# thvlio/bp-from-video

Hardware: NVIDIA B200
Metric: roi_sampled_frames_per_s (higher is better)
Workload: dtype f64

## Files before the change

bp-from-video_b200/csrc/window_pre.cu:

```cuda
#include <stdlib.h>
#include "filters.cuh"
#include "corr_tile.cuh"

namespace bpv {

int launch_job_butter(const double* ring_t, const bpv_window_params& p, double* sos_out, cudaStream_t st);
int launch_job_firls(const double* ring_t, const bpv_window_params& p, double* taps_out, cudaStream_t st);
int check_filter_params(const bpv_window_params* p, const char* who);
int launch_design_cached(const double* ring_t, const bpv_window_params& p, bool butter, bool fir, unsigned char* cache,
                         int32_t* ref, void* miss, double* ws_sos, double* ws_fir, cudaStream_t st);

struct DesignRef {
  const double* sos_ws;
  const double* taps_ws;
  const int32_t* ref;
  const unsigned char* cache;
  __device__ __forceinline__ const double* slot(long long job) const {
    const int sl = ref ? ref[job] : -1;
    return sl >= 0 ? reinterpret_cast<const double*>(cache + DC_HDR_BYTES + DC_SLOTS * 8) + (long long)sl * DC_STRIDE : nullptr;
  }
  __device__ __forceinline__ const double* sos(long long job) const {
    const double* v = slot(job);
    return v ? v : sos_ws + job * (MAX_SOS * 6);
  }
  __device__ __forceinline__ const double* fir(long long job) const {
    const double* v = slot(job);
    return v ? v + MAX_SOS * 6 : taps_ws + job * FIR_WS_STRIDE;
  }
};

struct PreLayout {
  int yv, xv, posv, posb, buf0, buf1, coef, total;
  int buf_len;
  int fir_c, fir_gt, fir_b;
};

__host__ __device__ inline int round_up(int v, int m) { return (v + m - 1) / m * m; }
__host__ __device__ inline int fir_ld_fwd(int n, int T) {
  int LD = (round_up(T, 8) + n + T + 15) / 8 + 1;
  LD += (6 - (LD & 3)) & 3;
  return LD;
}
__host__ __device__ inline int fir_ld_bwd(int n, int T) { return (round_up(T, 10) + n + T + 20) / 10 + 1; }
__host__ __device__ inline int fir_merged_k(int T, int RT) { return round_up(2 * T - 1, RT); }
__host__ __device__ inline int fir_merged_ld(int n, int T, int RT) { return (fir_merged_k(T, RT) / RT + (n + RT - 1) / RT) | 1; }

__host__ __device__ inline PreLayout pre_layout(const bpv_window_params& p, bool taps_global = false) {
  bool interp = false, cubic = false, butter = false, fir = false;
  for (int i = 0; i < p.num_methods; ++i) {
    const int m = p.methods[i];
    interp |= (m == BPV_INTERP_LINEAR || m == BPV_INTERP_CUBIC);
    cubic |= m == BPV_INTERP_CUBIC;
    butter |= m == BPV_FILTER_BUTTER;
    fir |= m == BPV_FILTER_FIR;
  }
  const int W = p.window;
  int pad = 0;
  if (butter) pad = 3 * (2 * p.butter_order + 1);
  if (pad > W - 1) pad = W - 1 > 0 ? W - 1 : 0;
  PreLayout L;
  L.buf_len = butter ? W + 2 * pad : (interp ? W : 0);
  L.fir_c = L.fir_gt = L.fir_b = 0;
  if (fir) {
    const int T = p.fir_taps, nf = W < T - 1 ? W : T - 1;
    L.fir_gt = 8 * fir_ld_fwd(nf, T);
    L.fir_b = L.fir_gt + 10 * fir_ld_bwd(nf, T);
    int need = L.fir_b;
    if (W >= T) {
      const int x8 = 8 * fir_merged_ld(W, T, 8), x10 = 10 * fir_merged_ld(W, T, 10);
      L.fir_c = ((x8 > x10 ? x8 : x10) + 1) & ~1;
      const int k8 = fir_merged_k(T, 8), k10 = fir_merged_k(T, 10);
      const int m = L.fir_c + (taps_global ? 0 : (k8 > k10 ? k8 : k10));
      if (m > need) need = m;
    }
    if (need > L.buf_len) L.buf_len = need;
  }
  int o = 0;
  auto sect = [&o](int bytes) { const int at = o; o += (bytes + 15) / 16 * 16; return at; };
  L.yv = sect(W * 8);
  L.xv = sect(interp ? W * 8 : 0);
  L.buf0 = sect(L.buf_len * 8);
  L.buf1 = sect(cubic ? W * 8 : 0);
  L.coef = sect(butter ? 128 * 8 : 0);
  L.posv = sect(W * 2);
  L.posb = sect(interp ? W * 2 : 0);
  L.total = o;
  return L;
}

__device__ __forceinline__ double shfl_d(double v, int src) { return __shfl_sync(0xffffffffu, v, src); }
__device__ __forceinline__ double shfl_up_d(double v, int d) { return __shfl_up_sync(0xffffffffu, v, d); }

struct Warp {
  int lane;
  double *yv, *xv, *buf0, *buf1, *coef;
  unsigned short *posv, *posb;
  int n, m;
  double xfirst, xlast;
  bool grid;
  int fir_c, fir_gt, fir_b;
  int W;
};

__device__ void diff1(Warp& w) {
  for (int c = (w.n - 1) / 32; c >= 0; --c) {
    const int i = c * 32 + w.lane;
    double v = 0.0;
    if (i < w.n && i > 0) v = w.yv[i] - w.yv[i - 1];
    __syncwarp();
    if (i < w.n) w.yv[i] = v;
    __syncwarp();
  }
}

__device__ void diff2(Warp& w) {
  const double y0 = w.yv[0], y1 = w.yv[1];
  __syncwarp();
  for (int c = (w.n - 1) / 32; c >= 0; --c) {
    const int i = c * 32 + w.lane;
    double v = 0.0;
    if (i < w.n) {
      const double z2 = w.yv[i];
      const double z1 = i >= 1 ? w.yv[i - 1] : y1;
      const double z0 = i >= 2 ? w.yv[i - 2] : (i == 1 ? y1 : y0);
      v = (z2 - z1) - (z1 - z0);
    }
    __syncwarp();
    if (i < w.n) w.yv[i] = v;
    __syncwarp();
  }
}

__device__ void detrend_const(Warp& w) {
  double s = 0.0;
  for (int i = w.lane; i < w.n; i += 32) s += w.yv[i];
  const double mean = warp_sum(s) / (double)w.n;
  for (int i = w.lane; i < w.n; i += 32) w.yv[i] -= mean;
  __syncwarp();
}

__device__ void detrend_linear(Warp& w) {
  const double N = (double)w.n, invN = 1.0 / N;
  double s = 0.0;
  for (int i = w.lane; i < w.n; i += 32) s += w.yv[i];
  const double ybar = warp_sum(s) * invN;
  const double ubar = (N + 1.0) * 0.5 * invN;
  double sxy = 0.0;
  for (int i = w.lane; i < w.n; i += 32) {
    const double du = fma((double)(i + 1), invN, -ubar);
    sxy = fma(du, w.yv[i] - ybar, sxy);
  }
  sxy = warp_sum(sxy);
  const double sxx = (N * N - 1.0) / (12.0 * N);
  const double slope = sxx > 0.0 ? sxy / sxx : 0.0;
  for (int i = w.lane; i < w.n; i += 32) {
    const double du = fma((double)(i + 1), invN, -ubar);
    w.yv[i] = (w.yv[i] - ybar) - slope * du;
  }
  __syncwarp();
}

__device__ __forceinline__ double grid_x(const Warp& w, int i, double step) {
  if (i == w.m - 1 && w.m > 1) return w.xlast;
  return __dadd_rn(__dmul_rn((double)i, step), w.xfirst);
}

__device__ __forceinline__ int bsearch_le(const double* xs, int n, double x) {
  int lo = 0, hi = n;
  while (hi - lo > 1) {
    const int mid = (lo + hi) >> 1;
    if (xs[mid] <= x) lo = mid; else hi = mid;
  }
  return lo;
}

__device__ void finish_interp(Warp& w, double step) {
  __syncwarp();
  for (int i = w.lane; i < w.m; i += 32) {
    w.yv[i] = w.buf0[i];
    w.xv[i] = grid_x(w, i, step);
    w.posv[i] = w.posb[i];
  }
  w.n = w.m;
  w.grid = true;
  __syncwarp();
}

__device__ void interp_linear(Warp& w) {
  const double step = (w.xlast - w.xfirst) / (double)(w.m - 1);
  const int n = w.n;
  for (int i = w.lane; i < w.m; i += 32) {
    const double xi = grid_x(w, i, step);
    double r;
    if (xi > w.xv[n - 1]) r = w.yv[n - 1];
    else if (xi < w.xv[0]) r = w.yv[0];
    else {
      const int j = bsearch_le(w.xv, n, xi);
      if (j == n - 1 || w.xv[j] == xi) r = w.yv[j];
      else {
        const double slope = (w.yv[j + 1] - w.yv[j]) / (w.xv[j + 1] - w.xv[j]);
        r = __dadd_rn(__dmul_rn(slope, xi - w.xv[j]), w.yv[j]);
      }
    }
    w.buf0[i] = r;
  }
  finish_interp(w, step);
}

__device__ bool interp_cubic(Warp& w) {
  const int n = w.n;
  const double* x = w.xv;
  const double* y = w.yv;
  int bad = 0;
  for (int i = w.lane; i + 1 < n; i += 32) bad |= !(x[i + 1] - x[i] > 0.0);
  if (__any_sync(0xffffffffu, bad)) return false;
  double* cp = w.buf0;
  double* s = w.buf1;
  if (w.lane == 0) {
    if (n == 2) {
      s[0] = s[1] = (y[1] - y[0]) / (x[1] - x[0]);
    } else if (n == 3) {
      const double dx0 = x[1] - x[0], dx1 = x[2] - x[1];
      const double sl0 = (y[1] - y[0]) / dx0, sl1 = (y[2] - y[1]) / dx1;
      const double s1 = (dx0 * sl1 + dx1 * sl0) / (dx0 + dx1);
      s[1] = s1; s[0] = 2.0 * sl0 - s1; s[2] = 2.0 * sl1 - s1;
    }
  }
  if (n > 3) {
    for (int i = 1 + w.lane; i <= n - 2; i += 32) {
      const double dxp = x[i] - x[i - 1], dxc = x[i + 1] - x[i];
      const double slp = (y[i] - y[i - 1]) / dxp, slc = (y[i + 1] - y[i]) / dxc;
      cp[i] = 2.0 * (dxp + dxc);
      s[i] = 3.0 * (dxc * slp + dxp * slc);
    }
    __syncwarp();
    if (w.lane == 0) {
      double cprev, sprev;
      {
        const double dx0 = x[1] - x[0], dx1 = x[2] - x[1];
        const double sl0 = (y[1] - y[0]) / dx0, sl1 = (y[2] - y[1]) / dx1;
        const double d = x[2] - x[0];
        const double rhs = ((dx0 + 2.0 * d) * dx1 * sl0 + dx0 * dx0 * sl1) / d;
        const double inv = 1.0 / dx1;
        cprev = d * inv; sprev = rhs * inv;
        cp[0] = cprev; s[0] = sprev;
      }
      double xm = x[0], xc = x[1], xn = x[2];
#pragma unroll 4
      for (int i = 1; i <= n - 2; ++i) {
        const double lo = xn - xc, up = xc - xm;
        const double inv = 1.0 / fma(-lo, cprev, cp[i]);
        cprev = up * inv;
        sprev = fma(-lo, sprev, s[i]) * inv;
        cp[i] = cprev; s[i] = sprev;
        xm = xc; xc = xn; xn = x[i + 2 < n ? i + 2 : n - 1];
      }
      {
        const double dxp = x[n - 2] - x[n - 3], dxc = x[n - 1] - x[n - 2];
        const double slp = (y[n - 2] - y[n - 3]) / dxp, slc = (y[n - 1] - y[n - 2]) / dxc;
        const double d = x[n - 1] - x[n - 3];
        const double rhs = (dxc * dxc * slp + (2.0 * d + dxc) * dxp * slc) / d;
        const double den = dxp - d * cprev;
        double sn = (rhs - d * sprev) / den;
        s[n - 1] = sn;
#pragma unroll 4
        for (int i = n - 2; i >= 0; --i) { sn = fma(-cp[i], sn, s[i]); s[i] = sn; }
      }
    }
  }
  __syncwarp();
  const double step = (w.xlast - w.xfirst) / (double)(w.m - 1);
  for (int i = w.lane; i < w.m; i += 32) {
    const double xi = grid_x(w, i, step);
    int j;
    if (xi < x[0]) j = 0;
    else if (xi >= x[n - 1]) j = n - 2;
    else j = bsearch_le(x, n, xi);
    const double dxj = x[j + 1] - x[j];
    const double slj = (y[j + 1] - y[j]) / dxj;
    const double t = (s[j] + s[j + 1] - 2.0 * slj) / dxj;
    const double c0 = t / dxj, c1 = (slj - s[j]) / dxj - t, c2 = s[j], c3 = y[j];
    const double u = xi - x[j];
    double res = c3, z = u;
    res = __dadd_rn(res, __dmul_rn(c2, z)); z = __dmul_rn(z, u);
    res = __dadd_rn(res, __dmul_rn(c1, z)); z = __dmul_rn(z, u);
    res = __dadd_rn(res, __dmul_rn(c0, z));
    cp[i] = res;
  }
  finish_interp(w, step);
  return true;
}

__device__ void odd_ext(const Warp& w, double* ext, int p) {
  const int n = w.n, L = n + 2 * p;
  const double y0 = w.yv[0], yl = w.yv[n - 1];
  for (int i = w.lane; i < L; i += 32) {
    double v;
    if (i < p) v = 2.0 * y0 - w.yv[p - i];
    else if (i < p + n) v = w.yv[i - p];
    else v = 2.0 * yl - w.yv[n - 2 - (i - p - n)];
    ext[i] = v;
  }
  __syncwarp();
}

__device__ void sos_filtfilt(Warp& w, const double* __restrict__ sos_g, int N) {
  double* sos = w.coef;
  double* zi = w.coef + 6 * MAX_SOS;
  for (int i = w.lane; i < N * 6; i += 32) sos[i] = sos_g[i];
  __syncwarp();
  int nb0 = 0, na0 = 0;
  if (w.lane == 0) {
    double scale = 1.0;
    for (int s = 0; s < N; ++s) {
      const double* c = sos + 6 * s;
      const double B0 = c[1] - c[4] * c[0], B1 = c[2] - c[5] * c[0];
      const double z0 = (B0 + B1) / (1.0 + c[4] + c[5]);
      zi[2 * s] = scale * z0;
      zi[2 * s + 1] = scale * (B1 - c[5] * z0);
      scale *= (c[0] + c[1] + c[2]) / (1.0 + c[4] + c[5]);
    }
  }
  for (int s = 0; s < N; ++s) { nb0 += sos[6 * s + 2] == 0.0; na0 += sos[6 * s + 5] == 0.0; }
  __syncwarp();
  const int dpl = 3 * (2 * N + 1 - (nb0 < na0 ? nb0 : na0));
  const int n = w.n, p = n <= dpl ? n - 1 : dpl;
  const int L = n + 2 * p;
  double* ext = w.buf0;
  odd_ext(w, ext, p);

  const int s = w.lane;
  const bool sec = s < N;
  const double b0 = sec ? sos[6 * s] : 0, b1 = sec ? sos[6 * s + 1] : 0, b2 = sec ? sos[6 * s + 2] : 0;
  const double a1 = sec ? sos[6 * s + 4] : 0, a2 = sec ? sos[6 * s + 5] : 0;
  const double zi0 = sec ? zi[2 * s] : 0, zi1 = sec ? zi[2 * s + 1] : 0;

  const double na1 = -a1, na2 = -a2;
  for (int pass = 0; pass < 2; ++pass) {
    const double x0 = pass == 0 ? ext[0] : ext[L - 1];
    double z0 = zi0 * x0, z1 = zi1 * x0;
    double prev_out = 0.0;
    const int dir = pass == 0 ? 1 : -1, base = pass == 0 ? 0 : L - 1;
    double nxt = ext[base];
    __syncwarp();
    const int t_steady = N - 1 < L ? N - 1 : L;
    int t = 0;
    for (; t < t_steady; ++t) {
      const double from_prev = shfl_up_d(prev_out, 1);
      const double xc = s == 0 ? nxt : from_prev;
      if (s == 0 && t + 1 < L) nxt = ext[base + dir * (t + 1)];
      if (sec && t >= s) {
        const double xn = fma(b0, xc, z0);
        z0 = fma(b1, xc, fma(na1, xn, z1));
        z1 = fma(b2, xc, na2 * xn);
        prev_out = xn;
      }
    }
    const double* in = ext + base + dir * (t + 1);
    double* out = ext + base + dir * (t - (N - 1));
    for (; t < L - 1; ++t) {
      const double from_prev = shfl_up_d(prev_out, 1);
      const double xc = s == 0 ? nxt : from_prev;
      if (s == 0) nxt = *in;
      in += dir;
      const double xn = fma(b0, xc, z0);
      z0 = fma(b1, xc, fma(na1, xn, z1));
      z1 = fma(b2, xc, na2 * xn);
      prev_out = xn;
      if (s == N - 1) *out = xn;
      out += dir;
    }
    for (; t < L + N - 1; ++t) {
      const double from_prev = shfl_up_d(prev_out, 1);
      const double xc = s == 0 ? nxt : from_prev;
      const int i = t - s;
      if (sec && i >= 0 && i < L) {
        const double xn = fma(b0, xc, z0);
        z0 = fma(b1, xc, fma(na1, xn, z1));
        z1 = fma(b2, xc, na2 * xn);
        prev_out = xn;
        if (s == N - 1) ext[base + dir * i] = xn;
      }
    }
    __syncwarp();
  }
  for (int i = w.lane; i < n; i += 32) w.yv[i] = ext[p + i];
  __syncwarp();
}

__device__ void sos_filtfilt_dual(Warp& wa, Warp& wb, bool la, bool lb, const double* __restrict__ ga,
                                  const double* __restrict__ gb, int N) {
  const int lane = wa.lane, hf = lane >> 4, s = lane & 15;
  const bool live = hf ? lb : la;
  double* yv = hf ? wb.yv : wa.yv;
  double* ext = hf ? wb.buf0 : wa.buf0;
  double* sos = hf ? wb.coef : wa.coef;
  double* zi = sos + 6 * MAX_SOS;
  const double* sg = hf ? gb : ga;
  const int n = live ? (hf ? wb.n : wa.n) : 0;
  if (live) for (int i = s; i < N * 6; i += 16) sos[i] = sg[i];
  __syncwarp();
  int nb0 = 0, na0 = 0;
  if (live) {
    if (s == 0) {
      double scale = 1.0;
      for (int k = 0; k < N; ++k) {
        const double* c = sos + 6 * k;
        const double B0 = c[1] - c[4] * c[0], B1 = c[2] - c[5] * c[0];
        const double z0 = (B0 + B1) / (1.0 + c[4] + c[5]);
        zi[2 * k] = scale * z0;
        zi[2 * k + 1] = scale * (B1 - c[5] * z0);
        scale *= (c[0] + c[1] + c[2]) / (1.0 + c[4] + c[5]);
      }
    }
    for (int k = 0; k < N; ++k) { nb0 += sos[6 * k + 2] == 0.0; na0 += sos[6 * k + 5] == 0.0; }
  }
  __syncwarp();
  const int dpl = 3 * (2 * N + 1 - (nb0 < na0 ? nb0 : na0));
  const int p = n <= dpl ? n - 1 : dpl;
  const int L = live ? n + 2 * p : 0;
  if (live) {
    const double y0 = yv[0], yl = yv[n - 1];
    for (int i = s; i < L; i += 16) {
      double v;
      if (i < p) v = 2.0 * y0 - yv[p - i];
      else if (i < p + n) v = yv[i - p];
      else v = 2.0 * yl - yv[n - 2 - (i - p - n)];
      ext[i] = v;
    }
  }
  __syncwarp();
  const int La = __shfl_sync(0xffffffffu, L, 0), Lb = __shfl_sync(0xffffffffu, L, 16);
  const int Lmax = La > Lb ? La : Lb;
  const int Lfast = (La > 0 && Lb > 0) ? (La < Lb ? La : Lb) : Lmax;
  const bool sec = live && s < N;
  const double b0 = sec ? sos[6 * s] : 0, b1 = sec ? sos[6 * s + 1] : 0, b2 = sec ? sos[6 * s + 2] : 0;
  const double a1 = sec ? sos[6 * s + 4] : 0, a2 = sec ? sos[6 * s + 5] : 0;
  const double zi0 = sec ? zi[2 * s] : 0, zi1 = sec ? zi[2 * s + 1] : 0;
  const double na1 = -a1, na2 = -a2;
  const bool first = live && s == 0, last = live && s == N - 1;
  for (int pass = 0; pass < 2; ++pass) {
    const double x0 = L > 0 ? (pass == 0 ? ext[0] : ext[L - 1]) : 0.0;
    double z0 = zi0 * x0, z1 = zi1 * x0;
    double prev_out = 0.0;
    const int dir = pass == 0 ? 1 : -1, base = pass == 0 ? 0 : L - 1;
    double nxt = L > 0 ? ext[base] : 0.0;
    __syncwarp();
    const int t_fill = N - 1 < Lmax ? N - 1 : Lmax;
    int t = 0;
    for (; t < t_fill; ++t) {
      const double from_prev = __shfl_up_sync(0xffffffffu, prev_out, 1, 16);
      const double xc = s == 0 ? nxt : from_prev;
      if (first && t + 1 < L) nxt = ext[base + dir * (t + 1)];
      if (sec && t >= s && t - s < L) {
        const double xn = fma(b0, xc, z0);
        z0 = fma(b1, xc, fma(na1, xn, z1));
        z1 = fma(b2, xc, na2 * xn);
        prev_out = xn;
        if (s == N - 1) ext[base + dir * (t - s)] = xn;
      }
    }
    if (Lfast > 0) {
      const double* in = ext + (L > 0 ? base + dir * (t + 1) : 0);
      double* out = ext + (L > 0 ? base + dir * (t - (N - 1)) : 0);
      for (; t < Lfast - 1; ++t) {
        const double from_prev = __shfl_up_sync(0xffffffffu, prev_out, 1, 16);
        const double xc = s == 0 ? nxt : from_prev;
        if (first) nxt = *in;
        in += dir;
        const double xn = fma(b0, xc, z0);
        z0 = fma(b1, xc, fma(na1, xn, z1));
        z1 = fma(b2, xc, na2 * xn);
        prev_out = xn;
        if (last) *out = xn;
        out += dir;
      }
    }
    for (; t < Lmax + N - 1; ++t) {
      const double from_prev = __shfl_up_sync(0xffffffffu, prev_out, 1, 16);
      const double xc = s == 0 ? nxt : from_prev;
      if (first && t + 1 < L) nxt = ext[base + dir * (t + 1)];
      const int i = t - s;
      if (sec && i >= 0 && i < L) {
        const double xn = fma(b0, xc, z0);
        z0 = fma(b1, xc, fma(na1, xn, z1));
        z1 = fma(b2, xc, na2 * xn);
        prev_out = xn;
        if (s == N - 1) ext[base + dir * i] = xn;
      }
    }
    __syncwarp();
  }
  if (live) for (int i = s; i < n; i += 16) yv[i] = ext[p + i];
  __syncwarp();
}

constexpr int FIR_RT = 8;
constexpr int FIR_RTB = 10;
__device__ void fir_filtfilt(Warp& w, const double* __restrict__ taps_g, int T) {
  const int Kp = (T + FIR_RT - 1) / FIR_RT * FIR_RT;
  const int KpB = (T + FIR_RTB - 1) / FIR_RTB * FIR_RTB;
  const double* __restrict__ b = taps_g;
  const double* __restrict__ zi = taps_g + 128;
  const int n = w.n, dpl = 3 * T, p = n <= dpl ? n - 1 : dpl;
  const int L = n + 2 * p;
  const int fa = p, fb = (p + n - 1 + T - 1) < (L - 1) ? (p + n - 1 + T - 1) : (L - 1);
  const int ba = p, bb = p + n - 1;
  const int xbase = fa - Kp, gbase = ba - KpB;
  int LD = (Kp + n + T + 15) / FIR_RT + 1;
  LD += (6 - (LD & 3)) & 3;
  const int LDB = (KpB + n + T + 2 * FIR_RTB) / FIR_RTB + 1;
  double* XT = w.buf0;
  double* GT = w.buf0 + w.fir_gt;
  const double y_first = w.yv[0], y_last = w.yv[n - 1];
#pragma unroll 3
  for (int jj = w.lane; jj < FIR_RT * LD; jj += 32) {
    const int i = jj + xbase;
    const bool inside = i >= 0 && i < L, head = i < p, tail = i >= p + n;
    const int src = head ? p - i : (tail ? 2 * n - 2 + p - i : i - p);
    const double y = w.yv[inside ? src : 0];
    const double v = head ? 2.0 * y_first - y : (tail ? 2.0 * y_last - y : y);
    XT[xt_index<FIR_RT>(jj, LD)] = inside ? v : 0.0;
  }
#pragma unroll 4
  for (int jj = w.lane; jj < FIR_RTB * LDB; jj += 32) GT[jj] = 0.0;
  __syncwarp();
  const double x0 = p >= 1 ? 2.0 * y_first - w.yv[p] : y_first;
  for (int I = Kp; I <= fb - xbase; I += 32 * FIR_RT) {
    const int j0 = I + FIR_RT * w.lane, i0 = j0 + xbase;
    if (i0 <= fb) {
      double acc[FIR_RT];
#pragma unroll
      for (int r = 0; r < FIR_RT; ++r) acc[r] = 0.0;
      corr_tile<FIR_RT, double, 0, 0, true>(acc, b, Kp, XT, LD, j0, 0, 0x7fffffff, T);
#pragma unroll
      for (int r = 0; r < FIR_RT; ++r) {
        const int i = i0 + r;
        if (i <= fb) {
          const double v = acc[r] + (i < T - 1 ? zi[i] * x0 : 0.0);
          const int g = L - 1 - i;
          GT[xt_index<FIR_RTB>(g - gbase, LDB)] = v;
        }
      }
    }
  }
  __syncwarp();
  const double yend = (0 - gbase >= 0) ? GT[xt_index<FIR_RTB>(0 - gbase, LDB)] : 0.0;
  for (int I = KpB; I <= bb - gbase; I += 32 * FIR_RTB) {
    const int j0 = I + FIR_RTB * w.lane, i0 = j0 + gbase;
    if (i0 <= bb) {
      double acc[FIR_RTB];
#pragma unroll
      for (int r = 0; r < FIR_RTB; ++r) acc[r] = 0.0;
      corr_tile<FIR_RTB, double, 0, 0, true>(acc, b, KpB, GT, LDB, j0, 0, 0x7fffffff, T);
#pragma unroll
      for (int r = 0; r < FIR_RTB; ++r) {
        const int i = i0 + r;
        if (i <= bb) w.yv[L - 1 - p - i] = acc[r] + (i < T - 1 ? zi[i] * yend : 0.0);
      }
    }
  }
  __syncwarp();
}

template <int RT, int LDC = 0, int KC = 0, bool CS = true>
__device__ void fir_merged(Warp& w, const double* __restrict__ c_g, int T) {
  const int M = T - 1;
  const int K = KC ? KC : fir_merged_k(T, RT);
  const int n = w.n, dpl = 3 * T, p = n <= dpl ? n - 1 : dpl;
  const int L = n + 2 * p;
  const int tiles = (n + RT - 1) / RT;
  const int LD = LDC ? LDC : fir_merged_ld(w.W, T, RT);
  double* XT = w.buf0;
  const double* c = c_g;
  if (CS) {
    double* cs = w.buf0 + w.fir_c;
    for (int k = w.lane; k < K; k += 32) cs[k] = c_g[k];
    c = cs;
  }
  const int xbase = p + M - K;
  const double y_first = w.yv[0], y_last = w.yv[n - 1];
  const int total = RT * (K / RT + tiles);
  const int j_h = xbase < 0 ? -xbase : 0;
  const int j_b = p - xbase, j_t = p + n - xbase;
  const int j_e = L - xbase < total ? L - xbase : total;
  for (int jj = w.lane; jj < j_h; jj += 32) XT[xt_index<RT>(jj, LD)] = 0.0;
  for (int jj = j_h + w.lane; jj < j_b; jj += 32) XT[xt_index<RT>(jj, LD)] = 2.0 * y_first - w.yv[j_b - jj];
  for (int jj = j_b + w.lane; jj < j_t && jj < total; jj += 32) XT[xt_index<RT>(jj, LD)] = w.yv[jj - j_b];
  for (int jj = j_t + w.lane; jj < j_e; jj += 32) XT[xt_index<RT>(jj, LD)] = 2.0 * y_last - w.yv[2 * n - 2 - (jj - j_b)];
  for (int jj = (j_e > j_t ? j_e : j_t) + w.lane; jj < total; jj += 32) XT[xt_index<RT>(jj, LD)] = 0.0;
  __syncwarp();
  for (int t = w.lane; t < tiles; t += 32) {
    double acc[RT];
#pragma unroll
    for (int r = 0; r < RT; ++r) acc[r] = 0.0;
    corr_tile<RT, double, LDC, KC>(acc, c, K, XT, LD, K + RT * t);
#pragma unroll
    for (int r = 0; r < RT; ++r) {
      const int m = RT * t + r;
      if (m < n) w.yv[m] = acc[r];
    }
  }
  __syncwarp();
}

template <bool CS>
__device__ __forceinline__ void fir_apply(Warp& w, const double* __restrict__ tg, int T) {
  const int n = w.n;
  if (n >= T) {
    const int c8 = ((n + 7) / 8 + 31) / 32 * 8 * fir_merged_k(T, 8);
    const int c10 = ((n + 9) / 10 + 31) / 32 * 10 * fir_merged_k(T, 10);
    const bool t127 = T == 127;
    if (c10 < c8) {
      if (t127 && w.W == 300) fir_merged<10, 57, 260, CS>(w, tg + 256, T);
      else fir_merged<10, 0, 0, CS>(w, tg + 256, T);
    } else {
      if (t127 && w.W == 300) fir_merged<8, 71, 256, CS>(w, tg + 256, T);
      else if (t127 && w.W == 250) fir_merged<8, 65, 256, CS>(w, tg + 256, T);
      else fir_merged<8, 0, 0, CS>(w, tg + 256, T);
    }
  } else {
    fir_filtfilt(w, tg, T);
  }
}

constexpr int F_INTERP = 1, F_BUTTER = 2, F_FIR = 4;
constexpr int F_TAPS_GLOBAL = 8;

__device__ __forceinline__ bool fs_is_finite(double xfirst, double xlast, int m) {
  const double d = fabs(xlast - xfirst);
  if (d > 1.0e-290 && d < 1.0e290) return true;
  return isfinite(1.0 / ((xlast - xfirst) / (double)(m - 1)));
}

template <int FEAT>
__device__ int gather_window(Warp& w, unsigned char* sm, const PreLayout& L, const bpv_window_params& p,
                             const double* __restrict__ ring_t, const double* __restrict__ ring_y, long long sig,
                             double* __restrict__ ox, double* __restrict__ oy) {
  bool has_interp = false;
  if (FEAT & F_INTERP)
    for (int i = 0; i < p.num_methods; ++i) has_interp |= (p.methods[i] == BPV_INTERP_LINEAR || p.methods[i] == BPV_INTERP_CUBIC);
  w.yv = reinterpret_cast<double*>(sm + L.yv);
  w.xv = reinterpret_cast<double*>(sm + L.xv);
  w.buf0 = reinterpret_cast<double*>(sm + L.buf0);
  w.buf1 = reinterpret_cast<double*>(sm + L.buf1);
  w.coef = reinterpret_cast<double*>(sm + L.coef);
  w.posv = reinterpret_cast<unsigned short*>(sm + L.posv);
  w.posb = reinterpret_cast<unsigned short*>(sm + L.posb);
  w.grid = false;
  w.W = p.window;
  w.fir_c = L.fir_c; w.fir_gt = L.fir_gt; w.fir_b = L.fir_b;
  const long long job = sig / p.R;
  const int r = (int)(sig % p.R);
  const int s = (int)(job / p.jobs_per_stream), j = (int)(job % p.jobs_per_stream);
  const long long head = p.head0 + (long long)j * p.head_step;
  const double* rt = ring_t + (long long)s * p.cap;
  const double* ry = ring_y + ((long long)s * p.R + r) * p.cap;
  const int W = p.window;
  int n = 0, m = 0;
  double xfirst = 0.0, xlast = 0.0;
  const unsigned lt = (1u << w.lane) - 1u;
  const long long gfirst = head - W + 1;
  const int kmin = gfirst < 0 ? (int)(-gfirst < W ? -gfirst : W) : 0;
  const int slot0 = (int)(((gfirst % p.cap) + p.cap) % p.cap);
  double* xstage = L.buf_len >= W ? w.buf0 : nullptr;
  bool allf = true;
  for (int k = w.lane; k < W; k += 32) {
    double x = nan_f64(), y = nan_f64();
    if (k >= kmin) { int slot = slot0 + k; if (slot >= p.cap) slot -= p.cap; x = rt[slot]; y = ry[slot]; }
    ox[k] = x; oy[k] = y;
    w.yv[k] = y;
    if (xstage) xstage[k] = x;
    allf &= isfinite(x) && isfinite(y);
  }
  __syncwarp();
  if (xstage && !has_interp && __all_sync(0xffffffffu, allf)) {
    for (int k = w.lane; k < W; k += 32) w.posv[k] = (unsigned short)k;
    w.n = w.m = W;
    w.xfirst = xstage[0]; w.xlast = xstage[W - 1];
    __syncwarp();
    return (W >= 2 && fs_is_finite(w.xfirst, w.xlast, W)) ? ST_OK : ST_GUARD;
  }
  for (int k0 = 0; k0 < W; k0 += 32) {
    const int k = k0 + w.lane;
    double x = nan_f64(), y = nan_f64();
    if (k < W) {
      y = w.yv[k];
      if (xstage) x = xstage[k];
      else if (k >= kmin) { int slot = slot0 + k; if (slot >= p.cap) slot -= p.cap; x = rt[slot]; }
    }
    const bool fx = isfinite(x), fy = isfinite(y);
    const unsigned bx = __ballot_sync(0xffffffffu, fx), by = __ballot_sync(0xffffffffu, fy);
    __syncwarp();
    if (fy) {
      const int idx = n + __popc(by & lt);
      w.yv[idx] = y; w.posv[idx] = (unsigned short)k;
      if (has_interp) w.xv[idx] = x;
    }
    if (fx && has_interp) w.posb[m + __popc(bx & lt)] = (unsigned short)k;
    if (bx) {
      if (m == 0) xfirst = shfl_d(x, __ffs(bx) - 1);
      xlast = shfl_d(x, 31 - __clz(bx));
    }
    __syncwarp();
    n += __popc(by); m += __popc(bx);
  }
  __syncwarp();
  w.n = n; w.m = m; w.xfirst = xfirst; w.xlast = xlast;
  return (n >= 2 && m >= 2 && fs_is_finite(xfirst, xlast, m)) ? ST_OK : ST_GUARD;
}

template <int FEAT>
__device__ int apply_method(Warp& w, int method, const bpv_window_params& p, const DesignRef& dr, long long job) {
  switch (method) {
    case BPV_DIFF_1: diff1(w); break;
    case BPV_DIFF_2: diff2(w); break;
    case BPV_INTERP_LINEAR: if (FEAT & F_INTERP) interp_linear(w); break;
    case BPV_INTERP_CUBIC: if (FEAT & F_INTERP) { if (!interp_cubic(w)) return ST_CUBIC_X; } break;
    case BPV_DETREND_CONST: detrend_const(w); break;
    case BPV_DETREND_LINEAR: detrend_linear(w); break;
    case BPV_FILTER_BUTTER:
      if (FEAT & F_BUTTER) {
        const double* sg = dr.sos(job);
        if (!isfinite(sg[0])) return ST_BAD_BANDS;
        sos_filtfilt(w, sg, p.butter_order);
      }
      break;
    case BPV_FILTER_FIR:
      if (FEAT & F_FIR) {
        const double* tg = dr.fir(job);
        if (!isfinite(tg[0])) return ST_BAD_BANDS;
        fir_apply<(FEAT & F_TAPS_GLOBAL) == 0>(w, tg, p.fir_taps);
      }
      break;
    default: break;
  }
  return ST_OK;
}

__device__ void scatter_window(const Warp& w, int st, int W, double* __restrict__ ox, double* __restrict__ oy,
                               int32_t* __restrict__ status, long long sig) {
  if (st == ST_OK) {
    for (int i = w.lane; i < w.n; i += 32) {
      const int k = w.posv[i];
      oy[k] = w.yv[i];
      if (w.grid) ox[k] = w.xv[i];
    }
  } else if (st != ST_GUARD) {
    for (int k = w.lane; k < W; k += 32) oy[k] = nan_f64();
  }
  if (w.lane == 0) status[sig] = st;
}

__device__ __forceinline__ void prefetch_filters(int FEAT, int lane, const bpv_window_params& p, const DesignRef& dr, long long job) {
  for (int i = 0; i < p.num_methods; ++i) {
    if ((FEAT & F_FIR) && p.methods[i] == BPV_FILTER_FIR) {
      asm volatile("prefetch.global.L1 [%0];" ::"l"(dr.fir(job) + lane * 16));
      if (lane == 0) asm volatile("prefetch.global.L1 [%0];" ::"l"(dr.fir(job) + 512));
    }
    if ((FEAT & F_BUTTER) && p.methods[i] == BPV_FILTER_BUTTER && lane * 16 < p.butter_order * 6)
      asm volatile("prefetch.global.L1 [%0];" ::"l"(dr.sos(job) + lane * 16));
  }
}

template <int FEAT, int MINB, bool DUAL>
__global__ void __launch_bounds__(128, MINB) window_preprocess_kernel(const double* __restrict__ ring_t,
                                                                      const double* __restrict__ ring_y,
                                                                      const bpv_window_params p, const PreLayout L,
                                                                      const DesignRef dr,
                                                                      double* __restrict__ proc_x, double* __restrict__ proc_y,
                                                                      int32_t* __restrict__ status) {
  extern __shared__ __align__(16) unsigned char smem_raw[];
  const int wib = threadIdx.x >> 5, wpb = blockDim.x >> 5;
  const long long unit = (long long)blockIdx.x * wpb + wib;
  const long long nsig = (long long)p.S * p.jobs_per_stream * p.R;
  const int W = p.window;
  const int lane = threadIdx.x & 31;
  if (!DUAL) {
    const long long sig = unit;
    if (sig >= nsig) return;
    Warp w;
    w.lane = lane;
    const long long job = sig / p.R;
    prefetch_filters(FEAT, lane, p, dr, job);
    double* ox = proc_x + sig * W;
    double* oy = proc_y + sig * W;
    int st = gather_window<FEAT>(w, smem_raw + (size_t)wib * L.total, L, p, ring_t, ring_y, sig, ox, oy);
    for (int mi = 0; mi < p.num_methods && st == ST_OK; ++mi) st = apply_method<FEAT>(w, p.methods[mi], p, dr, job);
    scatter_window(w, st, W, ox, oy, status, sig);
  } else {
    const long long sa = 2 * unit, sb = sa + 1;
    if (sa >= nsig) return;
    const bool hasb = sb < nsig;
    Warp wa, wb;
    wa.lane = wb.lane = lane;
    const long long ja = sa / p.R, jb = (hasb ? sb : sa) / p.R;
    prefetch_filters(FEAT, lane, p, dr, ja);
    if (jb != ja) prefetch_filters(FEAT, lane, p, dr, jb);
    unsigned char* sm = smem_raw + (size_t)wib * 2 * L.total;
    double* oxa = proc_x + sa * W; double* oya = proc_y + sa * W;
    double* oxb = proc_x + (hasb ? sb : sa) * W; double* oyb = proc_y + (hasb ? sb : sa) * W;
    int sta = gather_window<FEAT>(wa, sm, L, p, ring_t, ring_y, sa, oxa, oya);
    int stb = ST_GUARD;
    if (hasb) stb = gather_window<FEAT>(wb, sm + L.total, L, p, ring_t, ring_y, sb, oxb, oyb);
    else { wb = wa; }
    for (int mi = 0; mi < p.num_methods && (sta == ST_OK || stb == ST_OK); ++mi) {
      const int m = p.methods[mi];
      if (m == BPV_FILTER_BUTTER) {
        const double* ga = dr.sos(ja);
        const double* gb = dr.sos(jb);
        if (sta == ST_OK && !isfinite(ga[0])) sta = ST_BAD_BANDS;
        if (stb == ST_OK && !isfinite(gb[0])) stb = ST_BAD_BANDS;
        if (sta == ST_OK || stb == ST_OK) sos_filtfilt_dual(wa, wb, sta == ST_OK, stb == ST_OK, ga, gb, p.butter_order);
      } else {
        if (sta == ST_OK) sta = apply_method<FEAT & ~F_BUTTER>(wa, m, p, dr, ja);
        if (stb == ST_OK) stb = apply_method<FEAT & ~F_BUTTER>(wb, m, p, dr, jb);
      }
    }
    scatter_window(wa, sta, W, oxa, oya, status, sa);
    if (hasb) scatter_window(wb, stb, W, oxb, oyb, status, sb);
  }
}

template <int FEAT, int MINB, bool DUAL>
static int launch_preprocess(const double* ring_t, const double* ring_y, const bpv_window_params& p, const PreLayout& L,
                             const DesignRef& dr, double* proc_x, double* proc_y, int32_t* status, cudaStream_t st) {
  const int max_smem = 200 * 1024;
  const int per_warp = (DUAL ? 2 : 1) * L.total;
  BPV_REQUIRE(per_warp <= max_smem, BPV_E_TOO_LARGE, "bpv_window_preprocess: window %d needs %d B of shared memory per signal",
              p.window, L.total);
  const int reg_warps = MINB >= 6 ? 25 : (MINB == 5 ? 21 : 4 * MINB);
  int wpb = 1, best = 0;
  for (int c = 1; c <= 4; ++c) {
    const int per_block = c * per_warp + 1024;
    if (per_block > max_smem) break;
    int blocks = (227 * 1024) / per_block;
    if (blocks > 32) blocks = 32;
    int warps = blocks * c;
    if (warps > reg_warps) warps = reg_warps;
    if (warps > best || (warps == best && c < wpb)) { best = warps; wpb = c; }
  }
  const size_t smem = (size_t)wpb * per_warp;
  auto kern = window_preprocess_kernel<FEAT, MINB, DUAL>;
  if (int rc = ensure_dyn_smem((const void*)kern, smem)) return rc;
  const long long nsig = (long long)p.S * p.jobs_per_stream * p.R;
  const long long units = DUAL ? (nsig + 1) / 2 : nsig;
  kern<<<(unsigned)((units + wpb - 1) / wpb), wpb * 32, smem, st>>>(ring_t, ring_y, p, L, dr, proc_x, proc_y, status);
  return check_launch("bpv_window_preprocess");
}

static int parse_methods(const bpv_window_params* p, const char* who, bool& butter, bool& fir, bool& interp) {
  butter = fir = interp = false;
  BPV_REQUIRE(p->num_methods >= 0 && p->num_methods <= BPV_MAX_METHODS, BPV_E_INVALID, "%s: bad sizes", who);
  for (int i = 0; i < p->num_methods; ++i) {
    const int m = p->methods[i];
    BPV_REQUIRE(m >= BPV_DIFF_1 && m <= BPV_FILTER_FIR, BPV_E_UNSUPPORTED,
                "%s: unknown processing method %d (NotImplementedError, signal_processor.py:238)", who, m);
    butter |= m == BPV_FILTER_BUTTER;
    fir |= m == BPV_FILTER_FIR;
    interp |= m == BPV_INTERP_LINEAR || m == BPV_INTERP_CUBIC;
  }
  return 0;
}

}

namespace bpv {
struct WsPlan { long long sos, fir, ref, miss, total; };
static WsPlan ws_plan(const bpv_window_params* p) {
  const long long J = (long long)p->S * p->jobs_per_stream;
  WsPlan w;
  w.sos = 0;
  w.fir = w.sos + J * MAX_SOS * 6 * 8;
  w.ref = w.fir + J * FIR_WS_STRIDE * 8;
  w.miss = w.ref + (J * 4 + 7) / 8 * 8;
  w.total = w.miss + J * 16;
  return w;
}
}

extern "C" int64_t bpv_window_workspace_bytes(const bpv_window_params* p) {
  if (!p) return -1;
  return bpv::ws_plan(p).total;
}

extern "C" int64_t bpv_design_cache_bytes(void) { return bpv::DC_BYTES; }

extern "C" int bpv_window_design(const double* ring_t, const bpv_window_params* p, void* workspace, int64_t workspace_bytes,
                                 void* cache, int64_t cache_bytes, void* stream) {
  using namespace bpv;
  if (int rc = check_filter_params(p, "bpv_window_design")) return rc;
  BPV_REQUIRE(ring_t, BPV_E_INVALID, "bpv_window_design: NULL pointer");
  BPV_REQUIRE(p->S > 0 && p->window > 0 && p->window <= p->cap && p->jobs_per_stream > 0, BPV_E_INVALID, "bpv_window_design: bad sizes");
  bool butter, fir, interp;
  if (int rc = parse_methods(p, "bpv_window_design", butter, fir, interp)) return rc;
  if (!butter && !fir) return 0;
  const WsPlan wp = ws_plan(p);
  BPV_REQUIRE(workspace && workspace_bytes >= wp.total, BPV_E_INVALID,
              "bpv_window_design: workspace too small (see bpv_window_workspace_bytes)");
  BPV_REQUIRE(!cache || cache_bytes >= DC_BYTES, BPV_E_INVALID, "bpv_window_design: design cache too small (see bpv_design_cache_bytes)");
  unsigned char* ws = (unsigned char*)workspace;
  double* sos_ws = (double*)(ws + wp.sos);
  double* taps_ws = (double*)(ws + wp.fir);
  cudaStream_t st = (cudaStream_t)stream;
  if (cache)
    return launch_design_cached(ring_t, *p, butter, fir, (unsigned char*)cache, (int32_t*)(ws + wp.ref), ws + wp.miss, sos_ws, taps_ws, st);
  if (butter) if (int rc = launch_job_butter(ring_t, *p, sos_ws, st)) return rc;
  if (fir) if (int rc = launch_job_firls(ring_t, *p, taps_ws, st)) return rc;
  return 0;
}

extern "C" int bpv_window_filter(const double* ring_t, const double* ring_y, const bpv_window_params* p,
                                 const void* workspace, int64_t workspace_bytes, const void* cache, int64_t cache_bytes,
                                 double* proc_x, double* proc_y, int32_t* status, void* stream) {
  using namespace bpv;
  if (int rc = check_filter_params(p, "bpv_window_preprocess")) return rc;
  BPV_REQUIRE(ring_t && ring_y && proc_x && proc_y && status, BPV_E_INVALID, "bpv_window_preprocess: NULL pointer");
  BPV_REQUIRE(p->S > 0 && p->R > 0 && p->window > 0 && p->window <= p->cap && p->jobs_per_stream > 0, BPV_E_INVALID,
              "bpv_window_preprocess: bad sizes");
  BPV_REQUIRE(p->window <= 65535, BPV_E_TOO_LARGE, "bpv_window_preprocess: window > 65535");
  bool butter, fir, interp;
  if (int rc = parse_methods(p, "bpv_window_preprocess", butter, fir, interp)) return rc;
  const WsPlan wp = ws_plan(p);
  if (butter || fir) {
    BPV_REQUIRE(workspace && workspace_bytes >= wp.total, BPV_E_INVALID,
                "bpv_window_preprocess: workspace too small (see bpv_window_workspace_bytes)");
    BPV_REQUIRE(!cache || cache_bytes >= DC_BYTES, BPV_E_INVALID, "bpv_window_preprocess: design cache too small (see bpv_design_cache_bytes)");
  }
  const unsigned char* ws = (const unsigned char*)workspace;
  DesignRef dr;
  dr.sos_ws = ws ? (const double*)(ws + wp.sos) : nullptr;
  dr.taps_ws = ws ? (const double*)(ws + wp.fir) : nullptr;
  dr.ref = (ws && cache && (butter || fir)) ? (const int32_t*)(ws + wp.ref) : nullptr;
  dr.cache = (const unsigned char*)cache;
  static const bool taps_global = [] { const char* e = getenv("BPV_FIR_TAPS_GLOBAL"); return e && e[0] == '1'; }();
  const bool fir_only = !interp && !butter && fir;
  const PreLayout L = pre_layout(*p, fir_only && taps_global);
  cudaStream_t st = (cudaStream_t)stream;
#define BPV_PRE(feat, minb, dual) return launch_preprocess<feat, minb, dual>(ring_t, ring_y, *p, L, dr, proc_x, proc_y, status, st)
  const bool single_sos = getenv("BPV_SOS_SINGLE") != nullptr || (227 * 1024) / (2 * L.total + 1024) < 8;
  if (!interp && !butter && !fir) BPV_PRE(0, 6, false);
  if (fir_only && taps_global) BPV_PRE(F_FIR | F_TAPS_GLOBAL, 6, false);
  if (fir_only) BPV_PRE(F_FIR, 5, false);
  if (single_sos) {
    if (!interp && !fir) BPV_PRE(F_BUTTER, 4, false);
    BPV_PRE(F_INTERP | F_BUTTER | F_FIR, 4, false);
  }
  if (!interp && !fir) BPV_PRE(F_BUTTER, 4, true);
  if (!fir) BPV_PRE(F_INTERP | F_BUTTER, 4, true);
  BPV_PRE(F_INTERP | F_BUTTER | F_FIR, 4, true);
#undef BPV_PRE
}

extern "C" int bpv_window_preprocess(const double* ring_t, const double* ring_y, const bpv_window_params* p,
                                     void* workspace, int64_t workspace_bytes,
                                     double* proc_x, double* proc_y, int32_t* status, void* stream) {
  if (int rc = bpv_window_design(ring_t, p, workspace, workspace_bytes, nullptr, 0, stream)) return rc;
  return bpv_window_filter(ring_t, ring_y, p, workspace, workspace_bytes, nullptr, 0, proc_x, proc_y, status, stream);
}
```

Measured before the change: 23.67 million.

## Add chunked streaming FIR preprocessing kernel sharing overlapping windows per CTA

```diff
diff --git a/bp-from-video_b200/csrc/window_pre.cu b/bp-from-video_b200/csrc/window_pre.cu
--- a/bp-from-video_b200/csrc/window_pre.cu
+++ b/bp-from-video_b200/csrc/window_pre.cu
@@ -100,6 +100,7 @@
   bool grid;
   int fir_c, fir_gt, fir_b;
   int W;
+  const double* taps;
 };
 
 __device__ void diff1(Warp& w) {
@@ -563,7 +564,7 @@
   __syncwarp();
 }
 
-template <int RT, int LDC = 0, int KC = 0, bool CS = true>
+template <int RT, int LDC = 0, int KC = 0, bool CS = true, bool PRE = false>
 __device__ void fir_merged(Warp& w, const double* __restrict__ c_g, int T) {
   const int M = T - 1;
   const int K = KC ? KC : fir_merged_k(T, RT);
@@ -573,7 +574,9 @@
   const int LD = LDC ? LDC : fir_merged_ld(w.W, T, RT);
   double* XT = w.buf0;
   const double* c = c_g;
-  if (CS) {
+  if (PRE) {
+    c = w.taps;
+  } else if (CS) {
     double* cs = w.buf0 + w.fir_c;
     for (int k = w.lane; k < K; k += 32) cs[k] = c_g[k];
     c = cs;
@@ -604,7 +607,7 @@
   __syncwarp();
 }
 
-template <bool CS>
+template <bool CS, bool PRE = false>
 __device__ __forceinline__ void fir_apply(Warp& w, const double* __restrict__ tg, int T) {
   const int n = w.n;
   if (n >= T) {
@@ -612,12 +615,12 @@
     const int c10 = ((n + 9) / 10 + 31) / 32 * 10 * fir_merged_k(T, 10);
     const bool t127 = T == 127;
     if (c10 < c8) {
-      if (t127 && w.W == 300) fir_merged<10, 57, 260, CS>(w, tg + 256, T);
-      else fir_merged<10, 0, 0, CS>(w, tg + 256, T);
+      if (t127 && w.W == 300) fir_merged<10, 57, 260, CS, PRE>(w, tg + 256, T);
+      else fir_merged<10, 0, 0, CS, PRE>(w, tg + 256, T);
     } else {
-      if (t127 && w.W == 300) fir_merged<8, 71, 256, CS>(w, tg + 256, T);
-      else if (t127 && w.W == 250) fir_merged<8, 65, 256, CS>(w, tg + 256, T);
-      else fir_merged<8, 0, 0, CS>(w, tg + 256, T);
+      if (t127 && w.W == 300) fir_merged<8, 71, 256, CS, PRE>(w, tg + 256, T);
+      else if (t127 && w.W == 250) fir_merged<8, 65, 256, CS, PRE>(w, tg + 256, T);
+      else fir_merged<8, 0, 0, CS, PRE>(w, tg + 256, T);
     }
   } else {
     fir_filtfilt(w, tg, T);
@@ -626,6 +629,7 @@
 
 constexpr int F_INTERP = 1, F_BUTTER = 2, F_FIR = 4;
 constexpr int F_TAPS_GLOBAL = 8;
+constexpr int F_TAPS_CTA = 16;
 
 __device__ __forceinline__ bool fs_is_finite(double xfirst, double xlast, int m) {
   const double d = fabs(xlast - xfirst);
@@ -730,7 +734,7 @@
       if (FEAT & F_FIR) {
         const double* tg = dr.fir(job);
         if (!isfinite(tg[0])) return ST_BAD_BANDS;
-        fir_apply<(FEAT & F_TAPS_GLOBAL) == 0>(w, tg, p.fir_taps);
+        fir_apply<(FEAT & (F_TAPS_GLOBAL | F_TAPS_CTA)) == 0, (FEAT & F_TAPS_CTA) != 0>(w, tg, p.fir_taps);
       }
       break;
     default: break;
@@ -849,6 +853,158 @@
   return check_launch("bpv_window_preprocess");
 }
 
+constexpr int STREAM_WARPS = 4;
+
+struct StreamLayout {
+  int sx, sy;
+  int taps;
+  int posy, posx;
+  int ends;
+  int masks;
+  int refs;
+  int warps, slice;
+  int C, K, total;
+};
+
+static StreamLayout stream_layout(const bpv_window_params& p, const PreLayout& L, int C) {
+  StreamLayout S;
+  const int span = p.window + C - 1, nmask = span / 32 + 1;
+  int o = 0;
+  auto sect = [&o](int bytes) { const int at = o; o += (bytes + 15) / 16 * 16; return at; };
+  S.C = C;
+  const int k8 = fir_merged_k(p.fir_taps, 8), k10 = fir_merged_k(p.fir_taps, 10);
+  S.K = k8 > k10 ? k8 : k10;
+  S.sx = sect(span * 8);
+  S.sy = sect(span * 8);
+  S.taps = sect(S.K * 8);
+  S.posy = sect(span * 2);
+  S.posx = sect(span * 2);
+  S.ends = sect(4 * C * 4);
+  S.masks = sect(2 * nmask * 4);
+  S.refs = sect(C * 4);
+  S.slice = L.posv;
+  S.warps = sect(0);
+  S.total = S.warps + STREAM_WARPS * S.slice;
+  return S;
+}
+
+template <int MINB>
+__global__ void __launch_bounds__(32 * STREAM_WARPS, MINB) window_preprocess_stream_kernel(
+    const double* __restrict__ ring_t, const double* __restrict__ ring_y, const bpv_window_params p, const PreLayout L,
+    const StreamLayout SL, const DesignRef dr, double* __restrict__ proc_x, double* __restrict__ proc_y,
+    int32_t* __restrict__ status) {
+  extern __shared__ __align__(16) unsigned char smem_raw[];
+  constexpr int FEAT = F_FIR | F_TAPS_CTA;
+  const int tid = threadIdx.x, lane = tid & 31, wib = tid >> 5, nthr = 32 * STREAM_WARPS;
+  const int W = p.window, J = p.jobs_per_stream, C = SL.C;
+  const int nchunk = (J + C - 1) / C;
+  const int chunk = (int)(blockIdx.x % nchunk);
+  const int sr = (int)(blockIdx.x / nchunk);
+  const int s = sr / p.R, r = sr % p.R;
+  const int j0 = chunk * C, nj = J - j0 < C ? J - j0 : C;
+  const int span = W + nj - 1;
+  const long long job0 = (long long)s * J + j0;
+  double* sx = reinterpret_cast<double*>(smem_raw + SL.sx);
+  double* sy = reinterpret_cast<double*>(smem_raw + SL.sy);
+  double* taps = reinterpret_cast<double*>(smem_raw + SL.taps);
+  unsigned short* posy = reinterpret_cast<unsigned short*>(smem_raw + SL.posy);
+  unsigned short* posx = reinterpret_cast<unsigned short*>(smem_raw + SL.posx);
+  int* ends = reinterpret_cast<int*>(smem_raw + SL.ends);
+  unsigned* mky = reinterpret_cast<unsigned*>(smem_raw + SL.masks);
+  const int nmask = span / 32 + 1;
+  unsigned* mkx = mky + nmask;
+  int* same_ref = reinterpret_cast<int*>(smem_raw + SL.refs);
+
+  const double* tap0 = dr.fir(job0) + 256;
+  for (int i = tid; i < nj; i += nthr) same_ref[i] = dr.fir(job0 + i) + 256 == tap0;
+  for (int i = tid; i < SL.K; i += nthr) taps[i] = tap0[i];
+  const long long gfirst = p.head0 + j0 - W + 1;
+  const int kmin = gfirst < 0 ? (int)(-gfirst < span ? -gfirst : span) : 0;
+  const int slot0 = (int)(((gfirst % p.cap) + p.cap) % p.cap);
+  const double* rt = ring_t + (long long)s * p.cap;
+  const double* ry = ring_y + ((long long)s * p.R + r) * p.cap;
+  for (int k = tid; k < span; k += nthr) {
+    double x = nan_f64(), y = nan_f64();
+    if (k >= kmin) { int slot = slot0 + k; if (slot >= p.cap) slot -= p.cap; x = rt[slot]; y = ry[slot]; }
+    sx[k] = x; sy[k] = y;
+  }
+  __syncthreads();
+  for (int c = wib; c < nmask; c += STREAM_WARPS) {
+    const int k = c * 32 + lane;
+    const unsigned by = __ballot_sync(0xffffffffu, k < span && isfinite(sy[k]));
+    const unsigned bx = __ballot_sync(0xffffffffu, k < span && isfinite(sx[k]));
+    if (lane == 0) { mky[c] = by; mkx[c] = bx; }
+  }
+  __syncthreads();
+  {
+    const unsigned lt = (1u << lane) - 1u;
+    for (int c = wib; c < nmask; c += STREAM_WARPS) {
+      int by0 = 0, bx0 = 0;
+      for (int q = 0; q < c; ++q) { by0 += __popc(mky[q]); bx0 += __popc(mkx[q]); }
+      const unsigned by = mky[c], bx = mkx[c];
+      const int k = c * 32 + lane;
+      const int iy = by0 + __popc(by & lt), ix = bx0 + __popc(bx & lt);
+      if ((by >> lane) & 1u) posy[iy] = (unsigned short)k;
+      if ((bx >> lane) & 1u) posx[ix] = (unsigned short)k;
+      if (k < nj) { ends[k] = iy; ends[2 * C + k] = ix; }
+      if (k >= W && k - W < nj) { ends[C + k - W] = iy; ends[3 * C + k - W] = ix; }
+    }
+  }
+  __syncthreads();
+
+  unsigned char* sm = smem_raw + SL.warps + (size_t)wib * SL.slice;
+  Warp w;
+  w.lane = lane;
+  w.yv = reinterpret_cast<double*>(sm + L.yv);
+  w.buf0 = reinterpret_cast<double*>(sm + L.buf0);
+  w.xv = w.buf1 = w.coef = w.buf0;
+  w.posb = posy;
+  w.grid = false;
+  w.W = W;
+  w.fir_c = L.fir_c; w.fir_gt = L.fir_gt; w.fir_b = L.fir_b;
+  for (int jj = wib; jj < nj; jj += STREAM_WARPS) {
+    const long long job = job0 + jj, sig = job * p.R + r;
+    if (lane == 0) asm volatile("prefetch.global.L1 [%0];" ::"l"(dr.fir(job)));
+    double* ox = proc_x + sig * W;
+    double* oy = proc_y + sig * W;
+    const int y0 = ends[jj], n = ends[C + jj] - y0, x0 = ends[2 * C + jj], m = ends[3 * C + jj] - x0;
+    if (n == W) {
+      for (int k = lane; k < W; k += 32) { const double y = sy[jj + k]; ox[k] = sx[jj + k]; oy[k] = y; w.yv[k] = y; }
+    } else {
+      for (int k = lane; k < W; k += 32) { ox[k] = sx[jj + k]; oy[k] = sy[jj + k]; }
+      for (int i = lane; i < n; i += 32) w.yv[i] = sy[posy[y0 + i]];
+    }
+    w.posv = posy + y0;
+    w.n = n; w.m = m;
+    w.xfirst = m > 0 ? sx[posx[x0]] : 0.0;
+    w.xlast = m > 0 ? sx[posx[x0 + m - 1]] : 0.0;
+    int st = (n >= 2 && m >= 2 && fs_is_finite(w.xfirst, w.xlast, m)) ? ST_OK : ST_GUARD;
+    w.taps = taps;
+    if (!same_ref[jj]) {
+      double* own = w.buf0 + w.fir_c;
+      if (st == ST_OK && n >= p.fir_taps) { const double* tg = dr.fir(job) + 256; for (int i = lane; i < SL.K; i += 32) own[i] = tg[i]; }
+      w.taps = own;
+    }
+    __syncwarp();
+    for (int mi = 0; mi < p.num_methods && st == ST_OK; ++mi) st = apply_method<FEAT>(w, p.methods[mi], p, dr, job);
+    const int sh = st == ST_OK ? jj : 0;
+    scatter_window(w, st, W, ox - sh, oy - sh, status, sig);
+    __syncwarp();
+  }
+}
+
+template <int MINB>
+static int launch_preprocess_stream(const double* ring_t, const double* ring_y, const bpv_window_params& p, const PreLayout& L,
+                                    const StreamLayout& SL, const DesignRef& dr, double* proc_x, double* proc_y,
+                                    int32_t* status, cudaStream_t st) {
+  auto kern = window_preprocess_stream_kernel<MINB>;
+  if (int rc = ensure_dyn_smem((const void*)kern, SL.total, true)) return rc;
+  const long long nchunk = (p.jobs_per_stream + SL.C - 1) / SL.C;
+  const long long ctas = (long long)p.S * p.R * nchunk;
+  kern<<<(unsigned)ctas, 32 * STREAM_WARPS, SL.total, st>>>(ring_t, ring_y, p, L, SL, dr, proc_x, proc_y, status);
+  return check_launch("bpv_window_preprocess");
+}
+
 static int parse_methods(const bpv_window_params* p, const char* who, bool& butter, bool& fir, bool& interp) {
   butter = fir = interp = false;
   BPV_REQUIRE(p->num_methods >= 0 && p->num_methods <= BPV_MAX_METHODS, BPV_E_INVALID, "%s: bad sizes", who);
@@ -941,6 +1097,17 @@
   const bool single_sos = getenv("BPV_SOS_SINGLE") != nullptr || (227 * 1024) / (2 * L.total + 1024) < 8;
   if (!interp && !butter && !fir) BPV_PRE(0, 6, false);
   if (fir_only && taps_global) BPV_PRE(F_FIR | F_TAPS_GLOBAL, 6, false);
+  if (fir_only && p->head_step == 1 && p->jobs_per_stream > 1) {
+    const char* es = getenv("BPV_F2_STREAM");
+    const char* ec = getenv("BPV_F2_CHUNK");
+    int C = ec && ec[0] ? atoi(ec) : 16;
+    C = C < 1 ? 1 : (C > 32 ? 32 : C);
+    const int span = p->window + (C < p->jobs_per_stream ? C : p->jobs_per_stream) - 1;
+    const PreLayout LS = pre_layout(*p);
+    const StreamLayout SL = stream_layout(*p, LS, C);
+    if (!(es && es[0] == '0') && span <= p->cap && span <= 65535 && SL.total <= 200 * 1024)
+      return launch_preprocess_stream<5>(ring_t, ring_y, *p, LS, SL, dr, proc_x, proc_y, status, st);
+  }
   if (fir_only) BPV_PRE(F_FIR, 5, false);
   if (single_sos) {
     if (!interp && !fir) BPV_PRE(F_BUTTER, 4, false);
```

Result: faster. 24.00 million, median of 6 (+1.4%).
